# rfahrn/RadVLM

Hardware: AMD Instinct MI355X
Metric: train image-instruction pairs/sec, LLaVA-1.5-7B 336px (higher is better)
Workload: dtype bf16; 1 GPU; llava15_7b full fine-tune step (ViT frozen): fwd+bwd+AdamW, S=704, 32 pairs/GPU/step; global_batch=32, seq_len=704, parallelism=dp1, rows_with_a_label_only=last layer's o_proj / norm / MLP, final norm, lm_head, cross entropy

## Files before the change

include/radvlm_hip.h:

```cpp
#ifndef RADVLM_HIP_H
#define RADVLM_HIP_H
#include <stdint.h>

#ifdef __cplusplus
extern "C" {
#endif

#define RV_ACT_NONE 0
#define RV_ACT_QUICK_GELU 1
#define RV_ACT_GELU 2
#define RV_ACT_GELU_TANH 3

const char* rv_version(void);

int rv_gemm_nt_bf16(const void* A, int64_t lda, const void* B, int64_t ldb, void* C, int64_t ldc, const void* bias,
                    const void* residual, int64_t ldr, int M, int N, int K, int act, int out_f32, int res_f32,
                    const void* zeros16, void* stream);
int rv_gemm_bf16(const void* A, int64_t lda, const void* B, int64_t ldb, void* C, int64_t ldc, const void* bias,
                 const void* residual, int64_t ldr, int M, int N, int K, int trans_a, int trans_b, float alpha, int act,
                 int out_f32, int res_f32, const void* zeros16, void* stream);
int rv_gemm_bf16_ex(const void* A, int64_t lda, const void* B, int64_t ldb, void* C, int64_t ldc, const void* bias,
                    const void* residual, int64_t ldr, int M, int N, int K, int trans_a, int trans_b, float alpha, int act,
                    int out_f32, int res_f32, const void* A2, int64_t lda2, const void* B2, int64_t ldb2, int K2,
                    void* workspace, int64_t workspace_bytes, const void* zeros16, void* stream);
int rv_gemm_rope_bf16(const void* A, int64_t lda, const void* B, int64_t ldb, void* C, int64_t ldc, const void* bias, int M, int N, int K,
                      const float* cos_sin, const int32_t* positions, int S, int rope_heads, int hd, void* workspace,
                      int64_t workspace_bytes, const void* zeros16, void* stream);
int rv_gemm_swiglu_fwd_bf16(const void* A, int64_t lda, const void* Wgu, int64_t ldb, void* GU, int64_t ldgu, void* ACT, int64_t ldact,
                            int M, int F, int K, void* workspace, int64_t workspace_bytes, const void* zeros16, void* stream);
int rv_gemm_swiglu_bwd_bf16(const void* dY, int64_t ldy, const void* Wd, int64_t ldw, const void* GU, int64_t ldgu, void* dGU, int64_t lddgu,
                            void* dact_scratch, int64_t ld_dact, int M, int F, int K, void* workspace, int64_t workspace_bytes,
                            const void* zeros16, void* stream);
int rv_gemm_select_kernel(int which);
int rv_gemm_set_cu_budget(int total_cus, int reserved_cus);

int rv_transpose_bf16(const void* in, int64_t in_ld, int64_t in_bs0, int64_t in_bs1, void* out, int64_t out_ld,
                      int64_t out_bs0, int64_t out_bs1, int R, int C, int R_pad, int nb0, int nb1, int perm32,
                      void* stream);

// ... 158 lines not shown
```

radvlm_amd/csrc/gemm_bf16.hip:

```cpp
#include <type_traits>
#include "common.h"
#include "radvlm_hip.h"
#include <stdlib.h>

namespace {

constexpr int BM = 128, BN = 128, BK = 64;
constexpr int STAGE_BYTES = (BM + BN) * BK * 2;
constexpr int NSTAGE = 2;

struct GemmParams {
    const bf16* A; const bf16* B; void* C; const bf16* bias; const void* R; const bf16* zeros;
    long lda, ldb, ldc, ldr;
    int M, N, K, act, out_f32, res_f32, tiles_m, tiles_n;
    float alpha;
    const bf16* A2; const bf16* B2; long lda2, ldb2; int K2;
    float* ws; int splits;
    int n_full;
    int pgrid;
    const float* rope_cs; const int* rope_pos; int rope_S, rope_cols, rope_hd;
    int F; bf16* C2; long ldc2; const bf16* G; long ldg;
    unsigned bytesA, bytesB;
    unsigned bytesA2, bytesB2;
    unsigned drop_thr; float drop_scale; unsigned long long drop_seed;
};
enum { EPI_NONE = 0, EPI_ROPE = 1, EPI_SWIGLU_FWD = 2, EPI_SWIGLU_BWD = 3 };

DEVINL float erf_as(float x) {
    const float ax = fabsf(x);
    const float t = __frcp_rn(1.f + 0.3275911f * ax);
    const float p = t * (0.254829592f + t * (-0.284496736f + t * (1.421413741f + t * (-1.453152027f + t * 1.061405429f))));
    const float r = 1.f - p * __expf(-ax * ax);
    return copysignf(r, x);
}
DEVINL float apply_act(float x, int act) {
    if (act == RV_ACT_QUICK_GELU) return x / (1.f + __expf(-1.702f * x));
    if (act == RV_ACT_GELU) return 0.5f * x * (1.f + erf_as(x * 0.70710678118654752f));
    if (act == RV_ACT_GELU_TANH) return x / (1.f + __expf(-1.5957691216057308f * (x + 0.044715f * x * x * x)));
    return x;
}

// ... 656 lines not shown
            const bf16x8 gv = *(const bf16x8*)(P.G + (long)m * P.ldg + n), uv = *(const bf16x8*)(P.G + (long)m * P.ldg + P.F + n);
            bf16* cp = (bf16*)P.C + (long)m * P.ldc;
            dswiglu(acc[i][2 * a], acc[i][2 * a + 1], gv, uv, cp + n, cp + P.F + n);
        });
    }
}

#ifdef RV_STAMPS
static long long* g_stamp_host = nullptr;
extern "C" int rv_debug_set_stamp_buffer(void* p) { g_stamp_host = (long long*)p; return 0; }
#define RV_STAMP(i) do { if (MODE == 0 && P.ws && threadIdx.x == 0) ((long long*)P.ws)[(long)blockIdx.x * 4 + (i)] = wall_clock64(); } while (0)
#else
#define RV_STAMP(i) do { } while (0)
#endif

template <bool TA, bool TB, int MODE, int EPI = EPI_NONE, bool BUF = false>
__global__ __launch_bounds__(512, 1) void gemm_kernel_256(GemmParams P) {
    extern __shared__ __attribute__((aligned(16))) char smem[];
    const int wid = wave_id(), lane = lane_id();
    const int wr = wid >> 2, wc = wid & 3;
    RV_STAMP(0);

    const int nwg = P.tiles_m * P.tiles_n;
    constexpr bool PERSIST = (MODE == 0 || MODE == 1 || MODE == 3) && BUF;
    int vtile = blockIdx.x, kslice = 0;
    bool sliced = MODE == 2;
    if (MODE == 2) { vtile = (int)blockIdx.x / P.splits; kslice = (int)blockIdx.x % P.splits; }
    if (MODE == 3 && (int)blockIdx.x >= (PERSIST ? P.pgrid : P.n_full)) {
        const int r = (int)blockIdx.x - (PERSIST ? P.pgrid : P.n_full);
        vtile = P.n_full + r / P.splits; kslice = r % P.splits; sliced = true;
    }
    int m0, n0, tn;
    auto coords = [&](int vt) {
        const int pid = xcd_remap(vt, nwg);
        constexpr int GROUP_M = RV_GROUP_M;
        const int per_group = GROUP_M * P.tiles_n;
        const int group = pid / per_group;
        const int first_m = group * GROUP_M;
        const int gsz = min(P.tiles_m - first_m, GROUP_M);
        tn = (pid % per_group) / gsz;
        m0 = (first_m + (pid % per_group) % gsz) * BM2;
        n0 = tn * BN2;
    };
    coords(vtile);

    f32x4 acc[8][4];

    const int nt1 = (P.K + BK - 1) / BK;
    const int t0 = sliced ? (int)((long)kslice * nt1 / P.splits) : 0;
// ... 17 lines not shown
    __amdgpu_buffer_rsrc_t rsA2, rsB2;
    HalfPlan plA2[2], plB2[2];
    if constexpr (BUF && MODE == 1) {
        rsA2 = __builtin_amdgcn_make_buffer_rsrc((void*)P.A2, 0, P.bytesA2, 0x00020000);
        rsB2 = __builtin_amdgcn_make_buffer_rsrc((void*)P.B2, 0, P.bytesB2, 0x00020000);
    }
    auto make_plans2 = [&]() {
#pragma unroll
        for (int h = 0; h < 2; ++h) {
            plA2[h] = plan_half<TA, false, 0>(P.lda2, m0 + h * 128, P.M, wid, lane, h, 0, P.bytesA2);
            plB2[h] = plan_half<TB, true, 0>(P.ldb2, n0 + h * 128, P.N, wid, lane, h, 0, P.bytesB2);
        }
    };
    if constexpr (BUF) make_plans();
    if constexpr (BUF && MODE == 1) make_plans2();
    const int kstepA = TA ? (int)(P.lda * BK * 2) : BK * 2, kstepB = TB ? (int)(P.ldb * BK * 2) : BK * 2;
    const int kstepA2 = TA ? (int)(P.lda2 * BK * 2) : BK * 2, kstepB2 = TB ? (int)(P.ldb2 * BK * 2) : BK * 2;
    auto stageA = [&](int t, int slot, int h, auto pair_tag) {
        constexpr int PAIR = decltype(pair_tag)::value;
        char* dst = smem + (slot * 2 + h) * HALF_BYTES;
        if constexpr (BUF) {
            if (MODE == 1 && (PAIR == 1 || (PAIR == 2 && t >= nt1))) stage_half_buf(rsA2, plA2[h], (t - nt1) * kstepA2, dst, wid);
            else stage_half_buf(rsA, plA[h], (t0 + t) * kstepA, dst, wid);
            return;
        }
        if (MODE == 1 && t >= nt1) stage_half<TA>(P.A2, P.lda2, m0 + h * 128, P.M, (t - nt1) * BK, P.K2, P.zeros, dst, wid, lane);
        else stage_half<TA>(P.A, P.lda, m0 + h * 128, P.M, (t0 + t) * BK, P.K, P.zeros, dst, wid, lane);
    };
    auto stageB = [&](int t, int h, auto pair_tag) {
        constexpr int PAIR = decltype(pair_tag)::value;
        char* dst = smem + B_RING_OFF + ((t & 1) * 2 + h) * HALF_BYTES;
// ... 68 lines not shown

    RV_STAMP(2);
    if (MODE == 3 && sliced) {
        float* slab = P.ws + ((long)(vtile - P.n_full) * P.splits + kslice) * (BM2 * BN2);
#pragma unroll
        for (int i = 0; i < 8; ++i)
#pragma unroll
            for (int a = 0; a < 2; ++a) {
                float* wp = slab + (wr * 128 + i * 16 + (lane & 15)) * BN2 + wc * 64 + 32 * a + 8 * (lane >> 4);
                *(f32x4*)wp = acc[i][2 * a];
                *(f32x4*)(wp + 4) = acc[i][2 * a + 1];
            }
        return;
    }
    const int m0e = m0, n0e = n0, tne = tn;
    bool more = false;
    if constexpr (PERSIST) {
        vt0 += MODE == 3 ? P.pgrid : (int)gridDim.x;
        more = !sliced && vt0 < (MODE == 3 ? P.n_full : nwg);
        if (more) {
            coords(vt0); make_plans();
            if constexpr (MODE == 1) make_plans2();
            stageA(0, 0, 0, P0); stageA(0, 0, 1, P0); stageB(0, 0, P0); stageB(0, 1, P0);
        }
    }
    if (EPI != EPI_NONE) epilogue_fused<EPI>(acc, P, m0e, tne, wr, wc, lane);
    else epilogue_256<MODE == 3 ? 0 : MODE>(acc, P, m0e, n0e, wr, wc, lane, kslice);
#ifdef RV_STAMPS
    asm volatile("s_waitcnt vmcnt(0)" ::: "memory");
#endif
    RV_STAMP(3);
    if (!more) break;
    } while (PERSIST);
}

__global__ void splitk_reduce_kernel(GemmParams P) {
    const long i = (long)blockIdx.x * blockDim.x + threadIdx.x;
    const long total = (long)P.M * P.N;
    if (i >= total) return;
    const int m = (int)(i / P.N), n = (int)(i % P.N);
    float s = 0.f;
    for (int k = 0; k < P.splits; ++k) s += P.ws[(long)k * total + i];
// ... 86 lines not shown
        }
        if (s + 1 < s1) store(s + 1, nxt);
        __syncthreads();
    }
#pragma unroll
    for (int i = 0; i < 4; ++i)
#pragma unroll
        for (int j = 0; j < 2; ++j)
#pragma unroll
            for (int r = 0; r < 4; ++r) {
                const int ar = 16 * i + 4 * g + r, col = c0 + wid * 32 + 16 * j + (lane & 15);
                if (ar < P.R && col < P.K) P.ws[((long)split * P.R + ar) * P.K + col] = acc[i][j][r];
            }
}

__global__ __launch_bounds__(256) void tail_reduce_kernel(GemmParams P) {
    const int nwg = P.tiles_m * P.tiles_n;
    const int tt = blockIdx.x >> 5;
    const int e = ((blockIdx.x & 31) * 256 + threadIdx.x) * 8;
    const int row = e >> 8, col = e & 255;
    const int pid = xcd_remap(P.n_full + tt, nwg);
    constexpr int GROUP_M = RV_GROUP_M;
    const int per_group = GROUP_M * P.tiles_n;
    const int group = pid / per_group;
    const int first_m = group * GROUP_M;
    const int gsz = min(P.tiles_m - first_m, GROUP_M);
    const int m = (first_m + (pid % per_group) % gsz) * BM2 + row;
    const int n = ((pid % per_group) / gsz) * BN2 + col;
    if (m >= P.M || n >= P.N) return;
    float v[8] = {0, 0, 0, 0, 0, 0, 0, 0};
    for (int k = 0; k < P.splits; ++k) {
        const float* sp = P.ws + ((long)tt * P.splits + k) * (BM2 * BN2) + row * BN2 + col;
        const f32x4 a = *(const f32x4*)sp, b = *(const f32x4*)(sp + 4);
#pragma unroll
        for (int r = 0; r < 4; ++r) { v[r] += a[r]; v[4 + r] += b[r]; }
    }
// ... 28 lines not shown
        if (P.R) x += P.res_f32 ? ((const float*)P.R)[(long)m * P.ldr + n + r] : bf2f(((const bf16*)P.R)[(long)m * P.ldr + n + r]);
        if (P.out_f32) ((float*)P.C)[(long)m * P.ldc + n + r] = x;
        else ((bf16*)P.C)[(long)m * P.ldc + n + r] = f2bf(x);
    }
}

}

static int g_tail_split = 1;
static int g_force_kernel = 0;
static int g_cus = 0;
static int g_cus_device = -1;
static int g_reserved_cus = -1;
static int g_no_buf = 0;
static int g_persist = 1;
extern "C" int rv_gemm_select_kernel(int which) {
    if (which >= 40) { g_persist = which == 41; return RV_OK; }
    if (which >= 30) { g_no_buf = which == 30; return RV_OK; }
    if (which >= 20) { g_tail_split = which - 20; return RV_OK; }
    g_force_kernel = which;
    return RV_OK;
}
extern "C" int rv_gemm_set_cu_budget(int total_cus, int reserved_cus) {
    int dev = 0;
    if (hipGetDevice(&dev) != hipSuccess) return RV_ERR_LAUNCH;
    if (total_cus <= 0) {
        int n = 0;
        if (hipDeviceGetAttribute(&n, hipDeviceAttributeMultiprocessorCount, dev) != hipSuccess) return RV_ERR_LAUNCH;
        total_cus = n;
    }
    g_cus_device = dev;
// ... 14 lines not shown
}

static bool buf_extents(GemmParams& P, int trans_a, int trans_b) {
    if ((P.K % BK) && !(trans_a && trans_b)) return false;
    const long ea = (trans_a ? (long)P.K : (long)P.M) * P.lda * 2, eb = (trans_b ? (long)P.K : (long)P.N) * P.ldb * 2;
    if (ea >= (1L << 31) || eb >= (1L << 31) || g_no_buf) return false;
    P.bytesA = (unsigned)ea; P.bytesB = (unsigned)eb;
    return true;
}
static bool buf_extents2(GemmParams& P, int trans_a, int trans_b) {
    if ((P.K2 % BK) && !(trans_a && trans_b)) return false;
    const long ea = (trans_a ? (long)P.K2 : (long)P.M) * P.lda2 * 2, eb = (trans_b ? (long)P.K2 : (long)P.N) * P.ldb2 * 2;
    if (ea >= (1L << 31) || eb >= (1L << 31)) return false;
    P.bytesA2 = (unsigned)ea; P.bytesB2 = (unsigned)eb;
    return true;
}
template <bool TA, bool TB, int MODE, bool BUF = false>
static void launch256m(const GemmParams& P, hipStream_t st) {
    static bool set = false;
    if (!set) { (void)hipFuncSetAttribute((const void*)gemm_kernel_256<TA, TB, MODE, EPI_NONE, BUF>, hipFuncAttributeMaxDynamicSharedMemorySize, LDS_BYTES2); set = true; }
    const int nwg = P.tiles_m * P.tiles_n;
    const int blocks = MODE == 2 ? nwg * P.splits : (MODE == 3 ? P.n_full + (nwg - P.n_full) * P.splits : nwg);
    int grid = blocks;
    GemmParams Q = P;
    Q.pgrid = MODE == 3 ? P.n_full : blocks;
    if (g_persist && BUF && (MODE == 0 || MODE == 1) && blocks > cu_budget()) { grid = cu_budget(); Q.pgrid = grid; }
    if (g_persist && BUF && MODE == 3 && P.n_full > cu_budget()) { Q.pgrid = cu_budget(); grid = Q.pgrid + (nwg - P.n_full) * P.splits; }
    hipLaunchKernelGGL((gemm_kernel_256<TA, TB, MODE, EPI_NONE, BUF>), dim3(grid), dim3(512), LDS_BYTES2, st, Q);
    if (MODE == 3) hipLaunchKernelGGL(tail_reduce_kernel, dim3((nwg - P.n_full) * 32), dim3(256), 0, st, P);
    if (MODE == 2) {
        const long total = (long)P.M * P.N;
        hipLaunchKernelGGL(splitk_reduce_kernel, dim3((unsigned)((total + 255) / 256)), dim3(256), 0, st, P);
    }
}
template <bool TA, bool TB>
static void launch256(GemmParams& P, int mode, hipStream_t st) {
    if (mode == 1) { if (buf_extents(P, TA, TB) && buf_extents2(P, TA, TB)) launch256m<TA, TB, 1, true>(P, st); else launch256m<TA, TB, 1>(P, st); }
    else if (mode == 2) { if (buf_extents(P, TA, TB)) launch256m<TA, TB, 2, true>(P, st); else launch256m<TA, TB, 2>(P, st); }
    else if (buf_extents(P, TA, TB)) { if (mode == 3) launch256m<TA, TB, 3, true>(P, st); else launch256m<TA, TB, 0, true>(P, st); }
    else if (mode == 3) launch256m<TA, TB, 3>(P, st);
    else launch256m<TA, TB, 0>(P, st);
}

static int gemm_ex_impl(const void* A, int64_t lda, const void* B, int64_t ldb, void* C, int64_t ldc, const void* bias,
// ... 3 lines not shown
    if (!A || !B || !C || !zeros16 || M <= 0 || N <= 0 || K <= 0) return RV_ERR_ARG;
    if ((lda & 7) || (ldb & 7)) return RV_ERR_ARG;
    if ((!trans_a && (K & 7)) || (trans_a && (M & 7)) || (!trans_b && (K & 7)) || (trans_b && (N & 7))) return RV_ERR_ARG;
    if (((uintptr_t)A | (uintptr_t)B | (uintptr_t)zeros16) & 15) return RV_ERR_ARG;
    const bool ext = A2 && B2 && K2 > 0;
    if (ext && ((lda2 & 7) || (ldb2 & 7) || (!trans_a && (K2 & 7)) || (!trans_b && (K2 & 7)) || (((uintptr_t)A2 | (uintptr_t)B2) & 15))) return RV_ERR_ARG;
    GemmParams P;
    P.A = (const bf16*)A; P.B = (const bf16*)B; P.C = C; P.bias = (const bf16*)bias; P.R = residual;
    P.zeros = (const bf16*)zeros16;
    P.lda = lda; P.ldb = ldb; P.ldc = ldc; P.ldr = ldr;
    P.M = M; P.N = N; P.K = K; P.act = act; P.out_f32 = out_f32; P.res_f32 = res_f32; P.alpha = alpha;
    P.A2 = (const bf16*)A2; P.B2 = (const bf16*)B2; P.lda2 = lda2; P.ldb2 = ldb2; P.K2 = ext ? K2 : 0;
    P.ws = (float*)workspace; P.splits = 1;
    P.drop_thr = drop_p > 0.f ? rv_dropout_thr16(drop_p) : 0u; P.drop_scale = drop_p > 0.f ? 1.f / (1.f - drop_p) : 1.f; P.drop_seed = drop_seed;
    const bool dropping = P.drop_thr != 0;
    static bool attr_set = false;
    if (!attr_set) {
        (void)hipFuncSetAttribute((const void*)gemm_nt_kernel, hipFuncAttributeMaxDynamicSharedMemorySize, NSTAGE * STAGE_BYTES);
        const char* e = getenv("RV_GEMM_KERNEL");
        if (e) g_force_kernel = atoi(e);
        attr_set = true;
    }
    const long tiles256 = (long)((M + BM2 - 1) / BM2) * ((N + BN2 - 1) / BN2);
    const int nt = (K + BK - 1) / BK;
    const int force = g_force_kernel;
    const int cus = cu_budget();
    int mode = ext ? 1 : 0;
    if (dropping) workspace = nullptr;
    if (!ext && workspace && tiles256 <= cus / 4 && nt >= 16) {
        int sp = (int)(cus / tiles256);
        if (sp > nt / 4) sp = nt / 4;
        if (sp > 32) sp = 32;
        if (sp >= 2 && (int64_t)sp * M * N * 4 <= workspace_bytes) { mode = 2; P.splits = sp; }
    }
    P.n_full = 0;
    if (mode == 0 && workspace && g_tail_split && tiles256 > cus) {
        const int rem = (int)(tiles256 % cus);
// ... 16 lines not shown
        if (trans_a) { if (trans_b) launch256<true, true>(P, mode, st); else launch256<true, false>(P, mode, st); }
        else { if (trans_b) launch256<false, true>(P, mode, st); else launch256<false, false>(P, mode, st); }
    } else {
        P.tiles_m = (M + BM - 1) / BM; P.tiles_n = (N + BN - 1) / BN;
        hipLaunchKernelGGL(gemm_nt_kernel, dim3(P.tiles_m * P.tiles_n), dim3(256), NSTAGE * STAGE_BYTES, st, P);
    }
    return rv_check_launch();
}

extern "C" int rv_gemm_bf16_ex(const void* A, int64_t lda, const void* B, int64_t ldb, void* C, int64_t ldc, const void* bias,
                               const void* residual, int64_t ldr, int M, int N, int K, int trans_a, int trans_b, float alpha,
                               int act, int out_f32, int res_f32, const void* A2, int64_t lda2, const void* B2, int64_t ldb2,
                               int K2, void* workspace, int64_t workspace_bytes, const void* zeros16, void* stream) {
    return gemm_ex_impl(A, lda, B, ldb, C, ldc, bias, residual, ldr, M, N, K, trans_a, trans_b, alpha, act, out_f32, res_f32, A2, lda2, B2, ldb2, K2,
                        workspace, workspace_bytes, zeros16, stream, 0.f, 0);
}

extern "C" int rv_gemm_dropout_add_bf16(const void* A, int64_t lda, const void* B, int64_t ldb, void* C, int64_t ldc, int M, int N, int K,
                                        int trans_b, float alpha, float p, uint64_t seed, int accumulate, const void* zeros16, void* stream) {
    if (p < 0.f || p >= 1.f || (N & 7) || (ldc & 7) || (((uintptr_t)C) & 15)) return RV_ERR_ARG;
    return gemm_ex_impl(A, lda, B, ldb, C, ldc, nullptr, accumulate ? C : nullptr, ldc, M, N, K, 0, trans_b, alpha, RV_ACT_NONE, 0, 0, nullptr, 0,
                        nullptr, 0, 0, nullptr, 0, zeros16, stream, p, seed);
}

extern "C" int rv_gemm_bf16(const void* A, int64_t lda, const void* B, int64_t ldb, void* C, int64_t ldc, const void* bias,
                            const void* residual, int64_t ldr, int M, int N, int K, int trans_a, int trans_b, float alpha,
                            int act, int out_f32, int res_f32, const void* zeros16, void* stream) {
    return rv_gemm_bf16_ex(A, lda, B, ldb, C, ldc, bias, residual, ldr, M, N, K, trans_a, trans_b, alpha, act, out_f32, res_f32,
                           nullptr, 0, nullptr, 0, 0, nullptr, 0, zeros16, stream);
}
// ... 135 lines not shown
```

radvlm_amd/engine.py:

```python
import math

import numpy as np
import torch

from . import ops
from .params import (LORA_TARGETS, VP, FlatParams, fast_random_init_, lm_param_shapes, lora_trainable_shapes, portable_init_,
                     vision_param_shapes)
from .splice import build_splice_plan, merged_feature_rows, shifted_labels

BF16 = torch.bfloat16


def _ru(x, m):
    return (x + m - 1) // m * m


class LlavaEngine:
    def __init__(self, geo, device="cuda", merge_type="flat", image_aspect_ratio="square", image_grid_pinpoints=None,
                 max_len=None, init="portable", seed=0, rms_eps=1e-5, rope_theta=10000.0, process_group=None,
                 bucket_layers=1, train_vision_tower=False, lora=None, packed="auto", freeze_lm=False, train_embed_tokens=False,
                 freeze_projector=False,
                 padding_side="right", force_grad_sync=False, recompute=False):
        self.geo = geo
        self.weights_version = 0
# ... 934 lines not shown
        last = self._dev((cu_q[1:] - 1).astype(np.int32))
        hN, _ = ops.rmsnorm_fwd(ops.gather_rows(last, d, x), self.W("model.norm.weight"), self.eps)
        logits = self._decode_linear(hN, self.W("lm_head.weight"), out_dtype=torch.float32)
        cache.lens = lens.copy()
        return cache, logits[:, :self.vocab]

    def _cross_entropy(self, logits, tgt, V, inv, gscale):
        from . import lib
        rows = logits.shape[0]
        loss_rows = torch.empty(rows, dtype=torch.float32, device=logits.device)
        lib.call("rv_cross_entropy", logits, logits.stride(0), tgt, loss_rows, logits, logits.stride(0), rows, V, inv * gscale)
        loss = torch.empty(1, dtype=torch.float32, device=logits.device)
        lib.call("rv_sum_f32", loss_rows, rows, inv, loss)
        return loss, loss_rows

    def _linear_bwd(self, dy, x, w, gw, need_dx=True, dx_out=None):
        acc = self.grad_accum_started
        if gw is not None:
            ops.gemm(dy, x, ta=True, tb=True, out=gw, residual=gw if acc else None)
        if need_dx:
            return ops.gemm(dy, w, tb=True, out=dx_out)
        return None

    def _lora_seed(self, i, lname):
        k = [t for t, _, _ in LORA_TARGETS].index(lname)
        return (self.lora_step * 1000003 + i * 131 + k) & 0x7FFFFFFFFFFFFFFF

    def _MODS_QKV(self, d):
        kvd = self.kvd
        return (("self_attn.q_proj", 0, d), ("self_attn.k_proj", d, d + kvd), ("self_attn.v_proj", d + kvd, d + 2 * kvd))

    def _lora_ws(self):
        if getattr(self, "_ws", None) is None:
# ... 63 lines not shown
        if c["head_idx"] is not None:
            back = np.full(M, -1, dtype=np.int32)
            back[c["head_idx"][:c["head_rows"]]] = np.arange(c["head_rows"], dtype=np.int32)
            back = self._dev(back)
            if not c["last_sel"]:
                dx = ops.gather_rows(back, d, dx)
        if not frozen_lm:
            self._bucket_done("lm_head.weight", "lm_head.weight")
            self._bucket_done("model.norm.weight", "model.norm.weight")
        for i in reversed(range(L)):
            a = c["layers"][i]
            if "h1" not in a:
                _, a = self._layer_forward(i, a["x"], c["geom"], rows=self._dev(c["head_idx"]) if (c["last_sel"] and i == L - 1) else None)
            lv, gv = self._layer_views(i), self._layer_views(i, self.grads)
            sv = a["lora"]
            if self.lora or not self.fused:
                dact = self._lm_linear_bwd(dx, a["act"], lv["down"], gv.get("down"), i, (("mlp.down_proj", 0, d),), sv)
                dgu = ops.swiglu_bwd(dact, a["gu"], F)
            else:
                self._linear_bwd(dx, a["act"], lv["down"], gv.get("down"), need_dx=False)
                dgu = ops.gemm_swiglu_bwd(dx, lv["down"], a["gu"], F)
            dh2 = self._lm_linear_bwd(dgu, a["h2"], lv["gu"], gv.get("gu"), i, (("mlp.gate_proj", 0, F), ("mlp.up_proj", F, 2 * F)), sv)
            ops.rmsnorm_bwd(dh2, a["x_mid"], lv["ln2"], a["rstd2"], dx=dx, dx_add=True, dw=gv.get("ln2"), dw_accumulate=acc)
            dattn = self._lm_linear_bwd(dx, a.get("attn_sel", a["attn"]), lv["o"], gv.get("o"), i, (("self_attn.o_proj", 0, d),), sv)
            if "attn_sel" in a:
                dattn, dx = ops.gather_rows(back, d, dattn), ops.gather_rows(back, d, dx)
            qkv = a["qkv"]
            dqkv = torch.empty_like(qkv)
            ops.attn_bwd(qkv[:, :d], qkv[:, d:d + kvd], qkv[:, d + kvd:], a["attn"], dattn, a["lse"], B, S, H, hd, s_pad, True,
                         lens=lens, dq=dqkv[:, :d], dk=dqkv[:, d:d + kvd], dv=dqkv[:, d + kvd:], kv_heads=Hkv, cu=cu,
                         rope=(cs, pos) if self.fused else None, delta=self._stat_buffer("delta", B, H, s_pad))
            if not self.fused:
                ops.rope_inplace(dqkv, cs, S, H + Hkv, hd, 1, -1, positions=pos)
            if "bqkv" in gv:
                ops.bias_grad(dqkv, out=gv["bqkv"], accumulate=acc)
            dh1 = self._lm_linear_bwd(dqkv, a["h1"], lv["qkv"], gv.get("qkv"), i, self._MODS_QKV(d), sv)
            ops.rmsnorm_bwd(dh1, a["x"], lv["ln1"], a["rstd1"], dx=dx, dx_add=True, dw=gv.get("ln1"), dw_accumulate=acc)
            c["layers"][i] = None
            p = f"model.layers.{i}."
            if self.freeze_lm:
                pass
            elif frozen_lm:
                self._bucket_done(p + "self_attn.q_proj.lora_A.weight", p + "mlp.down_proj.lora_B.weight")
            else:
                self._bucket_done(p + "input_layernorm.weight", p + "mlp.down_proj.weight")
        plan = c["plan"]
        dev = self.device
        n_rows = plan["n_feat_rows"]
        fpos = self._dev(plan["feat_pos"])
        dfeat = ops.gather_rows(fpos, d, dx)
        rs = plan.get("resample")
# ... 256 lines not shown
```

radvlm_amd/lib.py:

```python
import ctypes
import os

import torch

_HERE = os.path.dirname(os.path.abspath(__file__))
_LIB_PATH = os.path.join(_HERE, "libradvlm_hip.so")

_c_void_p = ctypes.c_void_p
_i64 = ctypes.c_int64
_i32 = ctypes.c_int
_f32 = ctypes.c_float

ACT_NONE, ACT_QUICK_GELU, ACT_GELU, ACT_GELU_TANH = 0, 1, 2, 3

_SIGS = {
    "rv_gemm_nt_bf16": [_c_void_p, _i64, _c_void_p, _i64, _c_void_p, _i64, _c_void_p, _c_void_p, _i64, _i32, _i32, _i32,
                        _i32, _i32, _i32, _c_void_p, _c_void_p],
    "rv_gemm_bf16": [_c_void_p, _i64, _c_void_p, _i64, _c_void_p, _i64, _c_void_p, _c_void_p, _i64, _i32, _i32, _i32, _i32, _i32,
                     _f32, _i32, _i32, _i32, _c_void_p, _c_void_p],
    "rv_gemm_bf16_ex": [_c_void_p, _i64, _c_void_p, _i64, _c_void_p, _i64, _c_void_p, _c_void_p, _i64, _i32, _i32, _i32, _i32, _i32,
                        _f32, _i32, _i32, _i32, _c_void_p, _i64, _c_void_p, _i64, _i32, _c_void_p, _i64, _c_void_p, _c_void_p],
    "rv_gemm_rope_bf16": [_c_void_p, _i64, _c_void_p, _i64, _c_void_p, _i64, _c_void_p, _i32, _i32, _i32, _c_void_p, _c_void_p, _i32, _i32, _i32,
                          _c_void_p, _i64, _c_void_p, _c_void_p],
    "rv_gemm_swiglu_fwd_bf16": [_c_void_p, _i64, _c_void_p, _i64, _c_void_p, _i64, _c_void_p, _i64, _i32, _i32, _i32, _c_void_p, _i64, _c_void_p,
                                _c_void_p],
    "rv_gemm_swiglu_bwd_bf16": [_c_void_p, _i64, _c_void_p, _i64, _c_void_p, _i64, _c_void_p, _i64, _c_void_p, _i64, _i32, _i32, _i32, _c_void_p,
                                _i64, _c_void_p, _c_void_p],
    "rv_dropout_bf16": [_c_void_p, _c_void_p, _i64, _f32, ctypes.c_uint64, _c_void_p],
    "rv_dropout_add_bf16": [_c_void_p, _c_void_p, _i64, _f32, ctypes.c_uint64, _c_void_p],
    "rv_gemm_dropout_add_bf16": [_c_void_p, _i64, _c_void_p, _i64, _c_void_p, _i64, _i32, _i32, _i32, _i32, _f32, _f32, ctypes.c_uint64, _i32, _c_void_p,
                                 _c_void_p],
    "rv_lora_a_grad_bf16": [_c_void_p, _i64, _c_void_p, _i64, _c_void_p, _i64, _i32, _i32, _i32, _f32, ctypes.c_uint64, _i32, _c_void_p, _i64, _c_void_p],
    "rv_lora_down_bf16": [_c_void_p, _i64, _c_void_p, _i64, _c_void_p, _i64, _i32, _i32, _i32, _f32, _f32, ctypes.c_uint64, _c_void_p, _c_void_p],
    "rv_transpose_bf16": [_c_void_p, _i64, _i64, _i64, _c_void_p, _i64, _i64, _i64, _i32, _i32, _i32, _i32, _i32, _i32, _c_void_p],
    "rv_rmsnorm_fwd": [_c_void_p, _c_void_p, _c_void_p, _c_void_p, _i32, _i32, _f32, _c_void_p],
    "rv_rmsnorm_bwd": [_c_void_p, _c_void_p, _c_void_p, _c_void_p, _c_void_p, _i32, _c_void_p, _i32, _i32, _i32, _c_void_p],
# ... 145 lines not shown
```

radvlm_amd/ops.py:

```python
import math

import torch

from . import lib
from .lib import ACT_GELU, ACT_GELU_TANH, ACT_NONE, ACT_QUICK_GELU

BF16 = torch.bfloat16


def _chk(t, dtype=BF16):
    assert t.is_cuda and t.dtype == dtype, (t.device, t.dtype)
    return t


def round_up(x, m):
    return (x + m - 1) // m * m


_WS = {}


def default_workspace(device):
    key = (device.type, device.index)
    if key not in _WS:
# ... 15 lines not shown
    assert out.shape == (M, N) and out.stride(1) == 1 and out.dtype in (BF16, torch.float32)
    if bias is not None:
        _chk(bias)
        assert bias.numel() == N and bias.is_contiguous()
    res_f32 = 0
    ldr = 0
    if residual is not None:
        assert residual.shape == (M, N) and residual.stride(1) == 1
        res_f32 = int(residual.dtype == torch.float32)
        ldr = residual.stride(0)
    lib.call("rv_gemm_nt_bf16", a, a.stride(0), b, b.stride(0), out, out.stride(0), bias, residual, ldr, M, N, K, act,
             int(out.dtype == torch.float32), res_f32, lib.zeros16(a.device))
    return out


def gemm(a, b, ta=False, tb=False, out=None, bias=None, residual=None, act=ACT_NONE, out_dtype=BF16, alpha=1.0, a2=None, b2=None,
         workspace=None):
    _chk(a), _chk(b)
    assert a.stride(1) == 1 and b.stride(1) == 1
    (K, M) = a.shape if ta else a.shape[::-1]
    (K2, N) = b.shape if tb else b.shape[::-1]
    assert K == K2, (a.shape, b.shape, ta, tb)
    if out is None:
        out = torch.empty(M, N, dtype=out_dtype, device=a.device)
    assert out.shape == (M, N) and out.stride(1) == 1 and out.dtype in (BF16, torch.float32)
    res_f32, ldr = 0, 0
    if residual is not None:
        assert residual.shape == (M, N) and residual.stride(1) == 1
        res_f32, ldr = int(residual.dtype == torch.float32), residual.stride(0)
    if bias is not None:
        assert bias.numel() == N and bias.is_contiguous()
    if workspace is None:
        workspace = default_workspace(a.device)
    K2 = 0
    if a2 is not None:
        _chk(a2), _chk(b2)
        assert a2.stride(1) == 1 and b2.stride(1) == 1
        (K2, M2) = a2.shape if ta else a2.shape[::-1]
        (K2b, N2) = b2.shape if tb else b2.shape[::-1]
        assert M2 == M and N2 == N and K2 == K2b
    ws_bytes = workspace.numel() * workspace.element_size() if workspace is not None else 0
    lib.call("rv_gemm_bf16_ex", a, a.stride(0), b, b.stride(0), out, out.stride(0), bias, residual, ldr, M, N, K, int(ta), int(tb),
             float(alpha), act, int(out.dtype == torch.float32), res_f32, a2, a2.stride(0) if a2 is not None else 0, b2,
             b2.stride(0) if b2 is not None else 0, K2, workspace, ws_bytes, lib.zeros16(a.device))
    return out


def gemm_rope(a, b, cos_sin, S, rope_heads, hd, bias=None, positions=None, out=None):
    _chk(a), _chk(b)
    M, K = a.shape
    N = b.shape[0]
    assert b.shape[1] == K and a.stride(1) == 1 and b.stride(1) == 1
    if out is None:
        out = torch.empty(M, N, dtype=BF16, device=a.device)
    assert out.shape == (M, N) and out.stride(1) == 1 and out.dtype == BF16
    ws = default_workspace(a.device)
# ... 691 lines not shown
```

Before: 43.27 pairs/s.

## Batch paired weight-gradient GEMMs into one grouped persistent launch

Adds a grouped GEMM kernel variant that takes up to four independent problems with the same K and maps a single tile range across them. The LM backward pass uses it to run the down_proj and gate/up weight gradients as one launch, and the o_proj and qkv weight gradients as another. Each input-gradient GEMM is then issued separately. The aim is to cut the partially filled last wave of each weight-gradient GEMM on the persistent grid and to save launch overhead. In exchange, the o_proj weight gradient is deferred, the kernel gains a per-tile problem lookup with buffer descriptors rebuilt per tile, and the fused swiglu-bwd path no longer folds these GEMMs together.

```diff
diff --git a/include/radvlm_hip.h b/include/radvlm_hip.h
--- a/include/radvlm_hip.h
+++ b/include/radvlm_hip.h
@@ -23,6 +23,8 @@
                     const void* residual, int64_t ldr, int M, int N, int K, int trans_a, int trans_b, float alpha, int act,
                     int out_f32, int res_f32, const void* A2, int64_t lda2, const void* B2, int64_t ldb2, int K2,
                     void* workspace, int64_t workspace_bytes, const void* zeros16, void* stream);
+int rv_gemm_grouped_bf16(const int64_t* desc, int count, float alpha, void* workspace, int64_t workspace_bytes, const void* zeros16,
+                         void* stream);
 int rv_gemm_rope_bf16(const void* A, int64_t lda, const void* B, int64_t ldb, void* C, int64_t ldc, const void* bias, int M, int N, int K,
                       const float* cos_sin, const int32_t* positions, int S, int rope_heads, int hd, void* workspace,
                       int64_t workspace_bytes, const void* zeros16, void* stream);
diff --git a/radvlm_amd/csrc/gemm_bf16.hip b/radvlm_amd/csrc/gemm_bf16.hip
--- a/radvlm_amd/csrc/gemm_bf16.hip
+++ b/radvlm_amd/csrc/gemm_bf16.hip
@@ -25,6 +25,29 @@
     unsigned drop_thr; float drop_scale; unsigned long long drop_seed;
 };
 enum { EPI_NONE = 0, EPI_ROPE = 1, EPI_SWIGLU_FWD = 2, EPI_SWIGLU_BWD = 3 };
+
+constexpr int RV_MAX_GROUP = 4;
+struct GroupProb {
+    const bf16* A; const bf16* B; void* C; const void* R;
+    long lda, ldb, ldc, ldr;
+    int M, N, tiles_m, tiles_n, tile0;
+    unsigned bytesA, bytesB;
+};
+struct GroupParams : GemmParams {
+    GroupProb prob[RV_MAX_GROUP];
+    int total_tiles;
+};
+DEVINL int group_select(const GroupParams& G, GemmParams& P, int vt) {
+    int p = 0;
+#pragma unroll
+    for (int i = 1; i < RV_MAX_GROUP; ++i) p += vt >= G.prob[i].tile0 ? 1 : 0;
+    const GroupProb& g = G.prob[p];
+    P.A = g.A; P.B = g.B; P.C = g.C; P.R = g.R;
+    P.lda = g.lda; P.ldb = g.ldb; P.ldc = g.ldc; P.ldr = g.ldr;
+    P.M = g.M; P.N = g.N; P.tiles_m = g.tiles_m; P.tiles_n = g.tiles_n;
+    P.bytesA = g.bytesA; P.bytesB = g.bytesB;
+    return vt - g.tile0;
+}
 
 DEVINL float erf_as(float x) {
     const float ax = fabsf(x);
@@ -711,14 +734,21 @@
 #define RV_STAMP(i) do { } while (0)
 #endif
 
-template <bool TA, bool TB, int MODE, int EPI = EPI_NONE, bool BUF = false>
-__global__ __launch_bounds__(512, 1) void gemm_kernel_256(GemmParams P) {
+template <bool GRP, class KP>
+DEVINL int launch_tiles(const KP& PK) {
+    if constexpr (GRP) return PK.total_tiles;
+    else return PK.tiles_m * PK.tiles_n;
+}
+template <bool TA, bool TB, int MODE, int EPI = EPI_NONE, bool BUF = false, bool GRP = false>
+__global__ __launch_bounds__(512, 1) void gemm_kernel_256(std::conditional_t<GRP, GroupParams, GemmParams> PK) {
+    static_assert(!GRP || (BUF && EPI == EPI_NONE && (MODE == 0 || MODE == 3)), "grouped launches: plain buffer-addressed whole tiles + the tail split");
+    std::conditional_t<GRP, GemmParams, const GemmParams&> P = PK;
     extern __shared__ __attribute__((aligned(16))) char smem[];
     const int wid = wave_id(), lane = lane_id();
     const int wr = wid >> 2, wc = wid & 3;
     RV_STAMP(0);
 
-    const int nwg = P.tiles_m * P.tiles_n;
+    const int nwg = launch_tiles<GRP>(PK);
     constexpr bool PERSIST = (MODE == 0 || MODE == 1 || MODE == 3) && BUF;
     int vtile = blockIdx.x, kslice = 0;
     bool sliced = MODE == 2;
@@ -729,7 +759,8 @@
     }
     int m0, n0, tn;
     auto coords = [&](int vt) {
-        const int pid = xcd_remap(vt, nwg);
+        if constexpr (GRP) vt = group_select(PK, P, vt);
+        const int pid = xcd_remap(vt, GRP ? P.tiles_m * P.tiles_n : nwg);
         constexpr int GROUP_M = RV_GROUP_M;
         const int per_group = GROUP_M * P.tiles_n;
         const int group = pid / per_group;
@@ -777,7 +808,7 @@
     };
     if constexpr (BUF) make_plans();
     if constexpr (BUF && MODE == 1) make_plans2();
-    const int kstepA = TA ? (int)(P.lda * BK * 2) : BK * 2, kstepB = TB ? (int)(P.ldb * BK * 2) : BK * 2;
+    std::conditional_t<GRP, int, const int> kstepA = TA ? (int)(P.lda * BK * 2) : BK * 2, kstepB = TB ? (int)(P.ldb * BK * 2) : BK * 2;
     const int kstepA2 = TA ? (int)(P.lda2 * BK * 2) : BK * 2, kstepB2 = TB ? (int)(P.ldb2 * BK * 2) : BK * 2;
     auto stageA = [&](int t, int slot, int h, auto pair_tag) {
         constexpr int PAIR = decltype(pair_tag)::value;
@@ -876,18 +907,24 @@
         return;
     }
     const int m0e = m0, n0e = n0, tne = tn;
+    std::conditional_t<GRP, const GemmParams, const GemmParams&> PE = P;
     bool more = false;
     if constexpr (PERSIST) {
         vt0 += MODE == 3 ? P.pgrid : (int)gridDim.x;
         more = !sliced && vt0 < (MODE == 3 ? P.n_full : nwg);
         if (more) {
             coords(vt0); make_plans();
+            if constexpr (GRP) {
+                rsA = __builtin_amdgcn_make_buffer_rsrc((void*)P.A, 0, P.bytesA, 0x00020000);
+                rsB = __builtin_amdgcn_make_buffer_rsrc((void*)P.B, 0, P.bytesB, 0x00020000);
+                kstepA = TA ? (int)(P.lda * BK * 2) : BK * 2; kstepB = TB ? (int)(P.ldb * BK * 2) : BK * 2;
+            }
             if constexpr (MODE == 1) make_plans2();
             stageA(0, 0, 0, P0); stageA(0, 0, 1, P0); stageB(0, 0, P0); stageB(0, 1, P0);
         }
     }
-    if (EPI != EPI_NONE) epilogue_fused<EPI>(acc, P, m0e, tne, wr, wc, lane);
-    else epilogue_256<MODE == 3 ? 0 : MODE>(acc, P, m0e, n0e, wr, wc, lane, kslice);
+    if (EPI != EPI_NONE) epilogue_fused<EPI>(acc, PE, m0e, tne, wr, wc, lane);
+    else epilogue_256<MODE == 3 ? 0 : MODE>(acc, PE, m0e, n0e, wr, wc, lane, kslice);
 #ifdef RV_STAMPS
     asm volatile("s_waitcnt vmcnt(0)" ::: "memory");
 #endif
@@ -1004,12 +1041,16 @@
             }
 }
 
-__global__ __launch_bounds__(256) void tail_reduce_kernel(GemmParams P) {
-    const int nwg = P.tiles_m * P.tiles_n;
+template <bool GRP = false>
+__global__ __launch_bounds__(256) void tail_reduce_kernel(std::conditional_t<GRP, GroupParams, GemmParams> PK) {
+    std::conditional_t<GRP, GemmParams, const GemmParams&> P = PK;
+    int nwg = P.tiles_m * P.tiles_n;
     const int tt = blockIdx.x >> 5;
     const int e = ((blockIdx.x & 31) * 256 + threadIdx.x) * 8;
     const int row = e >> 8, col = e & 255;
-    const int pid = xcd_remap(P.n_full + tt, nwg);
+    int vt = P.n_full + tt;
+    if constexpr (GRP) { vt = group_select(PK, P, vt); nwg = P.tiles_m * P.tiles_n; }
+    const int pid = xcd_remap(vt, nwg);
     constexpr int GROUP_M = RV_GROUP_M;
     const int per_group = GROUP_M * P.tiles_n;
     const int group = pid / per_group;
@@ -1068,7 +1109,9 @@
 static int g_reserved_cus = -1;
 static int g_no_buf = 0;
 static int g_persist = 1;
+static int g_group = 1;
 extern "C" int rv_gemm_select_kernel(int which) {
+    if (which >= 50) { g_group = which == 51; return RV_OK; }
     if (which >= 40) { g_persist = which == 41; return RV_OK; }
     if (which >= 30) { g_no_buf = which == 30; return RV_OK; }
     if (which >= 20) { g_tail_split = which - 20; return RV_OK; }
@@ -1113,6 +1156,16 @@
     if (ea >= (1L << 31) || eb >= (1L << 31)) return false;
     P.bytesA2 = (unsigned)ea; P.bytesB2 = (unsigned)eb;
     return true;
+}
+static void first_use() {
+    static bool done = false;
+    if (done) return;
+    (void)hipFuncSetAttribute((const void*)gemm_nt_kernel, hipFuncAttributeMaxDynamicSharedMemorySize, NSTAGE * STAGE_BYTES);
+    const char* e = getenv("RV_GEMM_KERNEL");
+    if (e) g_force_kernel = atoi(e);
+    e = getenv("RV_GEMM_GROUP");
+    if (e) g_group = atoi(e) != 0;
+    done = true;
 }
 template <bool TA, bool TB, int MODE, bool BUF = false>
 static void launch256m(const GemmParams& P, hipStream_t st) {
@@ -1126,7 +1179,7 @@
     if (g_persist && BUF && (MODE == 0 || MODE == 1) && blocks > cu_budget()) { grid = cu_budget(); Q.pgrid = grid; }
     if (g_persist && BUF && MODE == 3 && P.n_full > cu_budget()) { Q.pgrid = cu_budget(); grid = Q.pgrid + (nwg - P.n_full) * P.splits; }
     hipLaunchKernelGGL((gemm_kernel_256<TA, TB, MODE, EPI_NONE, BUF>), dim3(grid), dim3(512), LDS_BYTES2, st, Q);
-    if (MODE == 3) hipLaunchKernelGGL(tail_reduce_kernel, dim3((nwg - P.n_full) * 32), dim3(256), 0, st, P);
+    if (MODE == 3) hipLaunchKernelGGL(tail_reduce_kernel<false>, dim3((nwg - P.n_full) * 32), dim3(256), 0, st, P);
     if (MODE == 2) {
         const long total = (long)P.M * P.N;
         hipLaunchKernelGGL(splitk_reduce_kernel, dim3((unsigned)((total + 255) / 256)), dim3(256), 0, st, P);
@@ -1160,13 +1213,7 @@
     P.ws = (float*)workspace; P.splits = 1;
     P.drop_thr = drop_p > 0.f ? rv_dropout_thr16(drop_p) : 0u; P.drop_scale = drop_p > 0.f ? 1.f / (1.f - drop_p) : 1.f; P.drop_seed = drop_seed;
     const bool dropping = P.drop_thr != 0;
-    static bool attr_set = false;
-    if (!attr_set) {
-        (void)hipFuncSetAttribute((const void*)gemm_nt_kernel, hipFuncAttributeMaxDynamicSharedMemorySize, NSTAGE * STAGE_BYTES);
-        const char* e = getenv("RV_GEMM_KERNEL");
-        if (e) g_force_kernel = atoi(e);
-        attr_set = true;
-    }
+    first_use();
     const long tiles256 = (long)((M + BM2 - 1) / BM2) * ((N + BN2 - 1) / BN2);
     const int nt = (K + BK - 1) / BK;
     const int force = g_force_kernel;
@@ -1213,6 +1260,83 @@
                                int K2, void* workspace, int64_t workspace_bytes, const void* zeros16, void* stream) {
     return gemm_ex_impl(A, lda, B, ldb, C, ldc, bias, residual, ldr, M, N, K, trans_a, trans_b, alpha, act, out_f32, res_f32, A2, lda2, B2, ldb2, K2,
                         workspace, workspace_bytes, zeros16, stream, 0.f, 0);
+}
+
+static bool big_enough_for_256(int M, int N);
+template <bool TA, bool TB, int MODE>
+static void launch_grouped(GroupParams& G, hipStream_t st) {
+    static bool set = false;
+    if (!set) { (void)hipFuncSetAttribute((const void*)gemm_kernel_256<TA, TB, MODE, EPI_NONE, true, true>, hipFuncAttributeMaxDynamicSharedMemorySize, LDS_BYTES2); set = true; }
+    const int total = G.total_tiles, cus = cu_budget();
+    const int blocks = MODE == 3 ? G.n_full + (total - G.n_full) * G.splits : total;
+    int grid = blocks;
+    G.pgrid = MODE == 3 ? G.n_full : blocks;
+    if (g_persist && MODE == 0 && blocks > cus) { grid = cus; G.pgrid = grid; }
+    if (g_persist && MODE == 3 && G.n_full > cus) { G.pgrid = cus; grid = G.pgrid + (total - G.n_full) * G.splits; }
+    hipLaunchKernelGGL((gemm_kernel_256<TA, TB, MODE, EPI_NONE, true, true>), dim3(grid), dim3(512), LDS_BYTES2, st, G);
+    if (MODE == 3) hipLaunchKernelGGL(tail_reduce_kernel<true>, dim3((total - G.n_full) * 32), dim3(256), 0, st, G);
+}
+template <bool TA, bool TB>
+static void launch_grouped_form(GroupParams& G, hipStream_t st) {
+    if (G.splits > 1) launch_grouped<TA, TB, 3>(G, st); else launch_grouped<TA, TB, 0>(G, st);
+}
+
+extern "C" int rv_gemm_grouped_bf16(const int64_t* desc, int count, float alpha, void* workspace, int64_t workspace_bytes, const void* zeros16,
+                                    void* stream) {
+    if (!desc || count < 1 || count > RV_MAX_GROUP || !zeros16) return RV_ERR_ARG;
+    first_use();
+    const int cus = cu_budget();
+    hipStream_t st = (hipStream_t)stream;
+    auto fld = [&](int i, int k) { return desc[i * 16 + k]; };
+    GroupParams G{};
+    const int K = (int)fld(0, 10), ta = fld(0, 11) != 0, tb = fld(0, 12) != 0;
+    bool ok = g_group && count >= 2 && !g_no_buf && g_force_kernel != 1 && !(((uintptr_t)zeros16) & 15);
+    long total = 0;
+    for (int i = 0; ok && i < count; ++i) {
+        const int M = (int)fld(i, 8), N = (int)fld(i, 9);
+        GemmParams T{};
+        T.A = (const bf16*)fld(i, 0); T.lda = fld(i, 1); T.B = (const bf16*)fld(i, 2); T.ldb = fld(i, 3); T.M = M; T.N = N; T.K = K;
+        ok = fld(i, 10) == K && (fld(i, 11) != 0) == ta && (fld(i, 12) != 0) == tb && !fld(i, 13) && !(fld(i, 6) && fld(i, 14)) &&
+             T.A && T.B && fld(i, 4) && M > 0 && N > 0 && K > 0 && !(T.lda & 7) && !(T.ldb & 7) &&
+             !((ta ? M : K) & 7) && !((tb ? N : K) & 7) && !((((uintptr_t)T.A) | ((uintptr_t)T.B)) & 15) && buf_extents(T, ta, tb);
+        if (!ok) break;
+        GroupProb& g = G.prob[i];
+        g.A = T.A; g.B = T.B; g.C = (void*)fld(i, 4); g.R = (const void*)fld(i, 6);
+        g.lda = T.lda; g.ldb = T.ldb; g.ldc = fld(i, 5); g.ldr = fld(i, 7);
+        g.M = M; g.N = N; g.tiles_m = (M + BM2 - 1) / BM2; g.tiles_n = (N + BN2 - 1) / BN2; g.tile0 = (int)total;
+        g.bytesA = T.bytesA; g.bytesB = T.bytesB;
+        total += (long)g.tiles_m * g.tiles_n;
+        if (!ta && !tb && g_force_kernel != 2 && !big_enough_for_256(M, N)) ok = false;
+    }
+    if (ok && total <= cus && workspace && (K + BK - 1) / BK >= 16) {
+        for (int i = 0; i < count; ++i) if ((long)G.prob[i].tiles_m * G.prob[i].tiles_n <= cus / 4) ok = false;
+    }
+    if (total >= (1L << 30)) ok = false;
+    if (!ok) {
+        for (int i = 0; i < count; ++i) {
+            const int rc = gemm_ex_impl((const void*)fld(i, 0), fld(i, 1), (const void*)fld(i, 2), fld(i, 3), (void*)fld(i, 4), fld(i, 5), nullptr,
+                                        (const void*)fld(i, 6), fld(i, 7), (int)fld(i, 8), (int)fld(i, 9), (int)fld(i, 10), fld(i, 11) != 0, fld(i, 12) != 0,
+                                        alpha, RV_ACT_NONE, fld(i, 13) != 0, fld(i, 14) != 0, nullptr, 0, nullptr, 0, 0, workspace, workspace_bytes, zeros16,
+                                        stream, 0.f, 0);
+            if (rc != RV_OK) return rc;
+        }
+        return RV_OK;
+    }
+    for (int i = count; i < RV_MAX_GROUP; ++i) G.prob[i].tile0 = 0x7fffffff;
+    G.zeros = (const bf16*)zeros16; G.K = K; G.alpha = alpha; G.act = RV_ACT_NONE; G.drop_scale = 1.f;
+    G.ws = (float*)workspace; G.splits = 1; G.n_full = 0; G.total_tiles = (int)total;
+    const int nt = (K + BK - 1) / BK, rem = (int)(total % cus);
+    if (workspace && g_tail_split && rem > 0) {
+        int64_t sp = cus / rem;
+        if (sp > nt / 16) sp = nt / 16;
+        if (sp > 32) sp = 32;
+        const int64_t fit = workspace_bytes / ((int64_t)rem * BM2 * BN2 * 4);
+        if (sp > fit) sp = fit;
+        if (sp >= 2) { G.splits = (int)sp; G.n_full = (int)(total - rem); }
+    }
+    if (ta) { if (tb) launch_grouped_form<true, true>(G, st); else launch_grouped_form<true, false>(G, st); }
+    else { if (tb) launch_grouped_form<false, true>(G, st); else launch_grouped_form<false, false>(G, st); }
+    return rv_check_launch();
 }
 
 extern "C" int rv_gemm_dropout_add_bf16(const void* A, int64_t lda, const void* B, int64_t ldb, void* C, int64_t ldc, int M, int N, int K,
diff --git a/radvlm_amd/engine.py b/radvlm_amd/engine.py
--- a/radvlm_amd/engine.py
+++ b/radvlm_amd/engine.py
@@ -972,9 +972,11 @@
         lib.call("rv_sum_f32", loss_rows, rows, inv, loss)
         return loss, loss_rows
 
-    def _linear_bwd(self, dy, x, w, gw, need_dx=True, dx_out=None):
+    def _linear_bwd(self, dy, x, w, gw, need_dx=True, dx_out=None, group=None):
         acc = self.grad_accum_started
-        if gw is not None:
+        if gw is not None and group is not None:
+            ops.gemm(dy, x, ta=True, tb=True, out=gw, residual=gw if acc else None, group=group)
+        elif gw is not None:
             ops.gemm(dy, x, ta=True, tb=True, out=gw, residual=gw if acc else None)
         if need_dx:
             return ops.gemm(dy, w, tb=True, out=dx_out)
@@ -1068,15 +1070,23 @@
                 _, a = self._layer_forward(i, a["x"], c["geom"], rows=self._dev(c["head_idx"]) if (c["last_sel"] and i == L - 1) else None)
             lv, gv = self._layer_views(i), self._layer_views(i, self.grads)
             sv = a["lora"]
-            if self.lora or not self.fused:
+            paired = self.fused and not self.lora
+            if not paired:
                 dact = self._lm_linear_bwd(dx, a["act"], lv["down"], gv.get("down"), i, (("mlp.down_proj", 0, d),), sv)
                 dgu = ops.swiglu_bwd(dact, a["gu"], F)
-            else:
-                self._linear_bwd(dx, a["act"], lv["down"], gv.get("down"), need_dx=False)
+                dh2 = self._lm_linear_bwd(dgu, a["h2"], lv["gu"], gv.get("gu"), i, (("mlp.gate_proj", 0, F), ("mlp.up_proj", F, 2 * F)), sv)
+            else:
                 dgu = ops.gemm_swiglu_bwd(dx, lv["down"], a["gu"], F)
-            dh2 = self._lm_linear_bwd(dgu, a["h2"], lv["gu"], gv.get("gu"), i, (("mlp.gate_proj", 0, F), ("mlp.up_proj", F, 2 * F)), sv)
+                with ops.gemm_group(2) as grp:
+                    self._linear_bwd(dx, a["act"], lv["down"], gv.get("down"), need_dx=False, group=grp)
+                    self._linear_bwd(dgu, a["h2"], lv["gu"], gv.get("gu"), need_dx=False, group=grp)
+                dh2 = ops.gemm(dgu, lv["gu"], tb=True)
             ops.rmsnorm_bwd(dh2, a["x_mid"], lv["ln2"], a["rstd2"], dx=dx, dx_add=True, dw=gv.get("ln2"), dw_accumulate=acc)
-            dattn = self._lm_linear_bwd(dx, a.get("attn_sel", a["attn"]), lv["o"], gv.get("o"), i, (("self_attn.o_proj", 0, d),), sv)
+            if not paired:
+                dattn = self._lm_linear_bwd(dx, a.get("attn_sel", a["attn"]), lv["o"], gv.get("o"), i, (("self_attn.o_proj", 0, d),), sv)
+            else:
+                grp = ops.gemm_group(2)
+                dattn = self._linear_bwd(dx, a.get("attn_sel", a["attn"]), lv["o"], gv.get("o"), group=grp)
             if "attn_sel" in a:
                 dattn, dx = ops.gather_rows(back, d, dattn), ops.gather_rows(back, d, dx)
             qkv = a["qkv"]
@@ -1088,7 +1098,12 @@
                 ops.rope_inplace(dqkv, cs, S, H + Hkv, hd, 1, -1, positions=pos)
             if "bqkv" in gv:
                 ops.bias_grad(dqkv, out=gv["bqkv"], accumulate=acc)
-            dh1 = self._lm_linear_bwd(dqkv, a["h1"], lv["qkv"], gv.get("qkv"), i, self._MODS_QKV(d), sv)
+            if not paired:
+                dh1 = self._lm_linear_bwd(dqkv, a["h1"], lv["qkv"], gv.get("qkv"), i, self._MODS_QKV(d), sv)
+            else:
+                with grp:
+                    self._linear_bwd(dqkv, a["h1"], lv["qkv"], gv.get("qkv"), need_dx=False, group=grp)
+                dh1 = ops.gemm(dqkv, lv["qkv"], tb=True)
             ops.rmsnorm_bwd(dh1, a["x"], lv["ln1"], a["rstd1"], dx=dx, dx_add=True, dw=gv.get("ln1"), dw_accumulate=acc)
             c["layers"][i] = None
             p = f"model.layers.{i}."
diff --git a/radvlm_amd/lib.py b/radvlm_amd/lib.py
--- a/radvlm_amd/lib.py
+++ b/radvlm_amd/lib.py
@@ -20,6 +20,7 @@
                      _f32, _i32, _i32, _i32, _c_void_p, _c_void_p],
     "rv_gemm_bf16_ex": [_c_void_p, _i64, _c_void_p, _i64, _c_void_p, _i64, _c_void_p, _c_void_p, _i64, _i32, _i32, _i32, _i32, _i32,
                         _f32, _i32, _i32, _i32, _c_void_p, _i64, _c_void_p, _i64, _i32, _c_void_p, _i64, _c_void_p, _c_void_p],
+    "rv_gemm_grouped_bf16": [_c_void_p, _i32, _f32, _c_void_p, _i64, _c_void_p, _c_void_p],
     "rv_gemm_rope_bf16": [_c_void_p, _i64, _c_void_p, _i64, _c_void_p, _i64, _c_void_p, _i32, _i32, _i32, _c_void_p, _c_void_p, _i32, _i32, _i32,
                           _c_void_p, _i64, _c_void_p, _c_void_p],
     "rv_gemm_swiglu_fwd_bf16": [_c_void_p, _i64, _c_void_p, _i64, _c_void_p, _i64, _c_void_p, _i64, _i32, _i32, _i32, _c_void_p, _i64, _c_void_p,
diff --git a/radvlm_amd/ops.py b/radvlm_amd/ops.py
--- a/radvlm_amd/ops.py
+++ b/radvlm_amd/ops.py
@@ -53,8 +53,43 @@
     return out
 
 
+class gemm_group:
+    MAX = 4
+
+    def __init__(self, expect=None):
+        assert expect is None or 1 <= expect <= self.MAX
+        self.expect, self.items = expect, []
+
+    def add(self, desc, alpha, workspace, keep):
+        if self.items and (self.items[0][1] != alpha or self.items[0][2] is not workspace or len(self.items) == self.MAX):
+            self.close()
+        self.items.append((desc, alpha, workspace, keep))
+        if self.expect is not None and len(self.items) >= self.expect:
+            self.close()
+
+    def close(self):
+        items, self.items = self.items, []
+        if not items:
+            return
+        import ctypes
+        flat = [v for it in items for v in it[0]]
+        _, alpha, ws, keep = items[0]
+        lib.call("rv_gemm_grouped_bf16", (ctypes.c_int64 * len(flat))(*flat), len(items), float(alpha), ws,
+                 ws.numel() * ws.element_size(), lib.zeros16(keep[0].device))
+
+    def __enter__(self):
+        return self
+
+    def __exit__(self, exc_type, exc, tb):
+        if exc_type is None:
+            self.close()
+        else:
+            self.items = []
+        return False
+
+
 def gemm(a, b, ta=False, tb=False, out=None, bias=None, residual=None, act=ACT_NONE, out_dtype=BF16, alpha=1.0, a2=None, b2=None,
-         workspace=None):
+         workspace=None, group=None):
     _chk(a), _chk(b)
     assert a.stride(1) == 1 and b.stride(1) == 1
     (K, M) = a.shape if ta else a.shape[::-1]
@@ -79,6 +114,11 @@
         (K2b, N2) = b2.shape if tb else b2.shape[::-1]
         assert M2 == M and N2 == N and K2 == K2b
     ws_bytes = workspace.numel() * workspace.element_size() if workspace is not None else 0
+    if group is not None and bias is None and act == ACT_NONE and a2 is None:
+        group.add((a.data_ptr(), a.stride(0), b.data_ptr(), b.stride(0), out.data_ptr(), out.stride(0),
+                   0 if residual is None else residual.data_ptr(), ldr, M, N, K, int(ta), int(tb), int(out.dtype == torch.float32), res_f32, 0),
+                  float(alpha), workspace, (a, b, out, residual))
+        return out
     lib.call("rv_gemm_bf16_ex", a, a.stride(0), b, b.stride(0), out, out.stride(0), bias, residual, ldr, M, N, K, int(ta), int(tb),
              float(alpha), act, int(out.dtype == torch.float32), res_f32, a2, a2.stride(0) if a2 is not None else 0, b2,
              b2.stride(0) if b2 is not None else 0, K2, workspace, ws_bytes, lib.zeros16(a.device))
```

Result: no change. 43.52 pairs/s (median of 6 runs) (+0.6%).
